# Hagtaril/HiddenPose

Hardware: AMD Instinct MI355X
Metric: samples/sec (128x128x512 meas) fwd+bwd (higher is better)
Workload: dtype f32; 1 GPU; NlosPose train step (fwd+L2Joint+BCEDice loss+bwd+Adam), 128x128x512 transients, batch 4/GPU, fp32, random-init weights, weight gradients of the 3^3 / 4^3 convolutions (and of small 1^3 ones) on a second stream; global_batch=4, world_size=1, parallelism=dp1

## Files before the change

### hiddenpose_amd/_lib.py

```python
from __future__ import annotations

import ctypes as C
import os
import threading

_PKG = os.path.dirname(os.path.abspath(__file__))
LIB_PATH = os.path.join(_PKG, "libhiddenpose_hip.so")

_lock = threading.Lock()
_lib = None


class HiddenPoseHipError(RuntimeError):
    pass


_vp, _fp, _i, _sz, _d = C.c_void_p, C.c_void_p, C.c_int, C.c_size_t, C.c_double
SIGNATURES = {
    "hp_version": (_i, []),
    "hp_last_error_string": (C.c_char_p, []),
    "hp_profile_enable": (_i, [_i]),
    "hp_profile_reset": (_i, []),
    "hp_profile_count": (_i, []),
    "hp_profile_get": (_i, [_i, C.c_char_p, _i, C.POINTER(C.c_int64), C.POINTER(C.c_double)]),
    "hp_range_enable": (_i, [_i]),
    "hp_range_push": (_i, [C.c_char_p]),
    "hp_range_pop": (_i, []),
    "hp_range_start": (C.c_int64, [C.c_char_p]),
    "hp_range_stop": (_i, [C.c_int64]),
    "hp_lct_host_constants": (_i, [_i, _i, _d, _d, _vp, _vp, _vp, _vp, _vp, _vp]),
    "hp_lct_plan_create": (_i, [C.POINTER(_vp), _i, _i, _d, _d, _i, _i]),
    "hp_lct_plan_create_mode": (_i, [C.POINTER(_vp), _i, _i, _d, _d, _i, _i, _i]),
    "hp_lct_plan_destroy": (_i, [_vp]),
    "hp_laplacian5_forward": (_i, [_fp, _fp, _fp, C.c_long, _i, _i, _i, _vp]),
    "hp_laplacian5_backward": (_i, [_fp, _fp, _fp, C.c_long, _i, _i, _i, _vp]),
    "hp_lct_workspace_bytes": (_sz, [_vp, _i]),
    "hp_lct_forward": (_i, [_vp, _fp, _fp, _i, _vp, _sz, _vp]),
    "hp_lct_backward": (_i, [_vp, _fp, _fp, _i, _vp, _sz, _vp]),
    "hp_lct_plan_get_invpsf": (_i, [_vp, _vp, _vp]),
    "hp_conv3d_packed_weight_elems": (_sz, [_vp]),
    "hp_conv3d_pack_weight": (_i, [_vp, _fp, _fp, _fp, _vp]),
    "hp_conv3d_unpack_wgrad": (_i, [_vp, _fp, _fp, _vp]),
    "hp_conv3d_forward": (_i, [_vp, _fp, _fp, _fp, _fp, _vp, _vp]),
    "hp_conv3d_backward_data": (_i, [_vp, _fp, _fp, _fp, _fp, _vp]),
    "hp_conv3d_backward_data_masked": (_i, [_vp, _fp, _fp, _fp, _fp, _vp, _vp]),
    "hp_conv3d_backward_data_bnsums": (_i, [_vp, _fp, _fp, _fp, _fp, _vp, _fp, _fp, _fp, _fp, _fp, _i, _vp, _vp, C.POINTER(C.c_int), _vp]),
    "hp_bn_backward_presummed": (_i, [_fp, _fp, _fp, C.c_long, _i, _fp, _fp, _fp, _fp, _i, _i, _fp, _fp, _vp, _vp, _vp, _i, _vp]),
    "hp_conv3d_backward_weight": (_i, [_vp, _fp, _fp, _fp, _vp]),
    "hp_conv3d_backward_weight_split": (_i, [_vp, C.POINTER(C.c_long), C.POINTER(C.c_long)]),
    "hp_bn_train_finalize": (_i, [_vp, C.c_long, _i, C.c_float, C.c_float, _fp, _fp, _fp, _fp, _vp]),
    "hp_bn_train_finalize_counted": (_i, [_vp, C.c_long, _i, C.c_float, C.c_float, _fp, _fp, _fp, _fp, _vp, _vp]),
    "hp_bn_eval_stats": (_i, [_fp, _fp, _i, C.c_float, _fp, _fp, _vp]),
    "hp_bn_apply": (_i, [_fp, _fp, _fp, C.c_long, _i, _fp, _fp, _fp, _fp, _i, _vp, _i, _vp]),
    "hp_bn_apply_res_bn": (_i, [_fp, _fp, _fp, C.c_long, _i, _fp, _fp, _fp, _fp, _i, _vp, _fp, _fp, _fp, _fp, _i, _vp]),
    "hp_cast_f32_to_bf16": (_i, [_fp, _vp, C.c_long, _vp]),
    "hp_cast_bf16_to_f32": (_i, [_vp, _fp, C.c_long, _vp]),
    "hp_bn_backward_workspace_bytes": (_sz, [_i]),
    "hp_bn_backward_dual": (_i, [_fp, _vp, C.c_long, _i, _fp, _fp, _fp, _fp, _fp, _i, _fp, _fp, _fp, _fp, _fp, _fp, _fp, _i,
                                 _fp, _fp, _vp, _i, _vp]),
    "hp_bn_backward": (_i, [_fp, _fp, _fp, _fp, _fp, C.c_long, _i, _fp, _fp, _fp, _fp, _i, _i, _fp, _fp, _vp, _vp, _i, _vp]),
    "hp_maxpool3d_k3s2_forward": (_i, [_fp, _fp, _i, _i, _i, _i, _i, _vp]),
    "hp_maxpool3d_k3s2_backward": (_i, [_fp, _fp, _fp, _fp, _i, _i, _i, _i, _i, _vp]),
    "hp_layout_transpose": (_i, [_fp, _fp, _i, C.c_long, _i, _i, _vp]),
    "hp_stem_bn_pool_workspace_bytes": (_sz, [_i]),
    "hp_stem_bn_relu_pool_forward": (_i, [_fp, _fp, _i, _i, _i, _i, _i, _fp, _fp, _fp, _fp, _vp, _vp]),
    "hp_stem_bn_relu_pool_backward": (_i, [_fp, _fp, _fp, _fp, _i, _i, _i, _i, _i, _fp, _fp, _fp, _fp, _i, _fp, _fp, _vp, _vp]),
    "hp_dconv3_forward": (_i, [_fp, _fp, _fp, _fp, _i, _i, _i, _i, _i, _i, _i, _vp]),
    "hp_dconv3_forward_fused": (_i, [_fp, _fp, _fp, _fp, _fp, _vp, _i, _i, _i, _i, _i, _i, _i, C.c_float, _vp]),
    "hp_dconv3_backward_data_workspace_bytes": (_sz, [_i, _i, _i, _i, _i, _i]),
    "hp_dconv3_backward_data": (_i, [_fp, _fp, _fp, _i, _i, _i, _i, _i, _i, _i, _vp, _vp]),
    "hp_dconv3_forward_fused_p": (_i, [_fp, _fp, _fp, _fp, _fp, _vp, _i, _i, _i, _i, _i, _i, _i, C.c_float, _i, _vp]),
    "hp_dconv3_backward_data_p": (_i, [_fp, _fp, _fp, _i, _i, _i, _i, _i, _i, _i, _i, _vp, _vp]),
    "hp_dconv3_backward_weight_p": (_i, [_fp, _fp, _fp, _fp, _i, _i, _i, _i, _i, _i, _i, _i, _vp, _vp]),
    "hp_dconv3_backward_weight_workspace_bytes": (_sz, [_i, _i, _i, _i, _i, _i]),
    "hp_dconv3_backward_weight": (_i, [_fp, _fp, _fp, _fp, _i, _i, _i, _i, _i, _i, _i, _vp, _vp]),
    "hp_groupnorm_workspace_bytes": (_sz, [_i, _i]),
    "hp_groupnorm_relu_forward": (_i, [_fp, _fp, _i, _i, _i, C.c_long, _fp, _fp, C.c_float, _fp, _fp, _vp, _vp]),
    "hp_groupnorm_relu_forward_v2": (_i, [_fp, _fp, _i, _i, _i, C.c_long, _fp, _fp, C.c_float, _vp, _fp, _fp, _fp, _fp, _vp, _vp]),
    "hp_groupnorm_relu_backward_v2": (_i, [_fp, _fp, _fp, _i, _i, _i, C.c_long, _fp, _fp, _fp, _fp, _fp, _fp, _fp, _vp, _vp]),
    "hp_maxpool3d_k2_forward": (_i, [_fp, _fp, C.c_long, _i, _i, _i, _vp]),
# ... 148 lines not shown
```

### hiddenpose_amd/csrc/hp_internal.h

```cpp
#pragma once
#include <hip/hip_runtime.h>

#include "hp_host.h"

namespace hp {

#define HP_CHECK_HIP(expr)                                                              \
  do {                                                                                  \
    hipError_t _e = (expr);                                                             \
    if (_e != hipSuccess) {                                                             \
      ::hp::set_error("%s:%d: %s -> %s", __FILE__, __LINE__, #expr, hipGetErrorString(_e)); \
      return HP_ERR_HIP;                                                                \
    }                                                                                   \
  } while (0)

struct ProfScope {
  ProfScope(const char* name, hipStream_t st);
  ~ProfScope();
  int slot = -1;
  hipStream_t st = nullptr;
  hipEvent_t stop = nullptr;
};
#define HP_PROF(name, stream) ::hp::ProfScope _hp_prof_scope(name, stream)

constexpr int ATTN_JOINT_SPLITS = 32;
constexpr int ATTN_GROUPED_MAX_N = 64;
constexpr int ATTN_BWD_DQ_SPLITS = 32;
void launch_attn_bwd_joint_keys(const float* ws_dk, const float* ws_dv, float* dK, float* dV, int BH, int Ntok, int dh, int nj, int frames,
                                hipStream_t st);
void launch_attn_bwd_dq_joint(const float* Q, const float* K0, const float* V, const float* dout, const float* lse, const float* delta,
                              float* part, float* dQ, int BH, int heads, int dh, int Ntok, int nj, hipStream_t st);
void launch_attention_patch(const float* Q, const float* K, const float* V, float* out, float* lse, int B, int heads, int dh, int Ntok,
                            int nj, int n, int frames, hipStream_t st);
void launch_attention_joint_merge(const float* part, float* out, float* lse, int BH, int heads, int dh, int Ntok, int nj, int nsplit,
                                  hipStream_t st);
void launch_attn_bwd_delta(const float* out, const float* dout, float* delta, int B, int heads, int dh, int Ntok, hipStream_t st);
void launch_attn_bwd_dq_patch(const float* Q, const float* K, const float* V, const float* dout, const float* lse, const float* delta,
                              float* dQ, int BH, int heads, int dh, int Ntok, int nj, int n, int frames, hipStream_t st);
void launch_attn_bwd_dq_joint_merge(const float* part, float* dQ, int BH, int Ntok, int dh, int nj, int nsplit, hipStream_t st);
void launch_attention_patch16(const float* Q, const float* K, const float* V, float* out, float* lse, int B, int heads, int dh, int Ntok,
                              int nj, int n, int frames, int precision, hipStream_t st);
void launch_attn_bwd_dq_joint_masked(const float* Q, const float* K0, const float* V, const float* dout, const float* lse,
                                     const float* delta, float* part, float* dQ, int BH, int heads, int dh, int Ntok, int nj,
                                     const unsigned char* key_mask, hipStream_t st);
inline int attn_masked16_check(const char* who, int num_joints, int mask_patch_queries) {
  HP_REQUIRE(mask_patch_queries == 0 || mask_patch_queries == 1, "%s: mask_patch_queries must be 0 or 1", who);
  if (mask_patch_queries) {
    set_error("%s: mask_patch_queries 1 not built at a 16-bit precision (only the joint / class queries apply the mask there)", who);
    return HP_ERR_UNSUPPORTED;
  }
  if (num_joints == 0) {
    set_error("%s: num_joints 0 not built (with no joint / class key an all-masked group would have an empty key set)", who);
    return HP_ERR_UNSUPPORTED;
  }
  return HP_OK;
}

#ifdef __HIPCC__
__device__ __forceinline__ float4 hp_ld4(const void* p, long i, int half) {
  if (half) {
    const uint2 u = *reinterpret_cast<const uint2*>(reinterpret_cast<const unsigned short*>(p) + i);
    return make_float4(__uint_as_float(u.x << 16), __uint_as_float(u.x & 0xffff0000u), __uint_as_float(u.y << 16),
                       __uint_as_float(u.y & 0xffff0000u));
  }
  return *reinterpret_cast<const float4*>(reinterpret_cast<const float*>(p) + i);
}
__device__ __forceinline__ float hp_ld1(const void* p, long i, int half) {
  if (half) return __uint_as_float((unsigned)reinterpret_cast<const unsigned short*>(p)[i] << 16);
  return reinterpret_cast<const float*>(p)[i];
}
__device__ __forceinline__ unsigned short hp_f2bf(float v) {
  typedef __attribute__((ext_vector_type(2))) float hp_f32x2;
  typedef __attribute__((ext_vector_type(2))) __bf16 hp_bf16x2;
  const hp_bf16x2 h = __builtin_convertvector((hp_f32x2){v, 0.f}, hp_bf16x2);
  return __builtin_bit_cast(unsigned int, h) & 0xffffu;
}
__device__ __forceinline__ void hp_st4(void* p, long i, float4 v, int half) {
  if (half) {
    typedef __attribute__((ext_vector_type(2))) float hp_f32x2;
    typedef __attribute__((ext_vector_type(2))) __bf16 hp_bf16x2;
    const hp_bf16x2 lo = __builtin_convertvector((hp_f32x2){v.x, v.y}, hp_bf16x2);
    const hp_bf16x2 hi = __builtin_convertvector((hp_f32x2){v.z, v.w}, hp_bf16x2);
    *reinterpret_cast<uint2*>(reinterpret_cast<unsigned short*>(p) + i) =
        make_uint2(__builtin_bit_cast(unsigned int, lo), __builtin_bit_cast(unsigned int, hi));
    return;
  }
  *reinterpret_cast<float4*>(reinterpret_cast<float*>(p) + i) = v;
}
__device__ __forceinline__ unsigned hp_extent(long total, long base_off, int esz) {
  const long bytes = (total - base_off) * esz;
// ... 10 lines not shown
```

### hiddenpose_amd/csrc/norm_kernels.hip

```cpp
#include <algorithm>
#include <cstdint>
#include <cstdlib>
#include <initializer_list>

#include "hp_internal.h"

namespace hp {

constexpr int ET = 256;
#ifndef HP_BN_UNR_H
#define HP_BN_UNR_H 8
#endif

#ifndef HP_BN_NT
#define HP_BN_NT 1
#endif
typedef float hp_f4v __attribute__((ext_vector_type(4)));
typedef unsigned hp_u4v __attribute__((ext_vector_type(4)));
__device__ __forceinline__ float4 ld_stream(const float4* p) {
#if HP_BN_NT
  const hp_f4v t = __builtin_nontemporal_load(reinterpret_cast<const hp_f4v*>(p));
  return make_float4(t.x, t.y, t.z, t.w);
#else
  return *p;
// ... 1077 lines not shown
  }
  hipLaunchKernelGGL(k_bn_bwd_coef, dim3((C + 127) / 128), dim3(128), 0, st, red, M, C, mean, rstd, gamma, train, dgamma,
                     dbeta, ca, cb, cc);
  {
    HP_PROF("bn_bwd_apply", st);
    const long n4 = M * C4;
    if (bytemask) {
      const int iom = io_mode(C4, {dy_half, z_half, dz_half});
      HP_LAUNCH_IOM(k_bn_bwd_apply_bytemask, iom, grid_for_bwd(n4 / (iom == 1 ? 2 : 1)), st, dy, dy_half, z, z_half, dz, dz_half, n4, C4,
                    (const float4*)ca, (const float4*)cb, (const float4*)cc, relu_mask);
    } else if (remask) {
      const int iom = io_mode(C4, {dy_half, z_half, dz_half});
      HP_LAUNCH_IOM(k_bn_bwd_apply_mask, iom, grid_for_bwd(n4 / (iom == 1 ? 2 : 1)), st, dy, dy_half, z, z_half, dz, dz_half, n4, C4,
                    (const float4*)ca, (const float4*)cb, (const float4*)cc, (const float4*)mean, (const float4*)rstd,
                    (const float4*)gamma, (const float4*)beta_for_mask, relu);
    } else {
      const int iom = io_mode(C4, {z_half, dz_half});
      HP_LAUNCH_IOM(k_bn_bwd_apply, iom, grid_for_bwd(n4 / (iom == 1 ? 2 : 1)), st, (const void*)gbuf, dz_half, z, z_half, dz, dz_half, n4,
                    C4, (const float4*)ca, (const float4*)cb, (const float4*)cc);
    }
  }
  HP_CHECK_HIP(hipGetLastError());
  return HP_OK;
}

__global__ void k_bn_sum_slots(const double* __restrict__ slots, double* __restrict__ red, int n) {
  const int i = blockIdx.x * blockDim.x + threadIdx.x;
  if (i >= n) return;
  double s = 0.0;
  for (int sl = 0; sl < HP_STATS_SLOTS; ++sl) s += slots[(size_t)sl * n + i];
  red[i] = s;
}

extern "C" int hp_bn_backward_presummed(const void* dy, const void* z, void* dz, long M, int C, const float* mean,
                                        const float* rstd, const float* gamma, const float* beta_for_mask, int relu, int train,
                                        float* dgamma, float* dbeta, const unsigned char* relu_mask, const double* sums,
                                        void* workspace, int io, void* stream) {
  const int dy_half = (io & HP_BN_DY_BF16) ? 1 : 0, dz_half = (io & HP_BN_DZ_BF16) ? 1 : 0, z_half = (io & HP_BN_Z_BF16) ? 1 : 0;
  HP_REQUIRE(dy && z && dz && mean && rstd && gamma && sums && workspace && M > 0 && C > 0 && C % 4 == 0 && dy != dz,
             "hp_bn_backward_presummed: bad argument");
  HP_REQUIRE(!relu || relu_mask || beta_for_mask, "hp_bn_backward_presummed: relu needs the byte mask, or beta to rebuild the mask from z");
  hipStream_t st = (hipStream_t)stream;
  double* red = (double*)workspace;
  float* ca = (float*)(red + 2 * C);
  float* cb = ca + C;
  float* cc = cb + C;
  const int C4 = C / 4;
  hipLaunchKernelGGL(k_bn_sum_slots, dim3((2 * C + 127) / 128), dim3(128), 0, st, sums, red, 2 * C);
  hipLaunchKernelGGL(k_bn_bwd_coef, dim3((C + 127) / 128), dim3(128), 0, st, red, M, C, mean, rstd, gamma, train, dgamma,
                     dbeta, ca, cb, cc);
  {
    HP_PROF("bn_bwd_apply", st);
    const long n4 = M * C4;
    const int iom = io_mode(C4, {dy_half, z_half, dz_half});
    if (relu && relu_mask)
      HP_LAUNCH_IOM(k_bn_bwd_apply_bytemask, iom, grid_for_bwd(n4 / (iom == 1 ? 2 : 1)), st, dy, dy_half, z, z_half, dz, dz_half, n4, C4,
                    (const float4*)ca, (const float4*)cb, (const float4*)cc, relu_mask);
    else
      HP_LAUNCH_IOM(k_bn_bwd_apply_mask, iom, grid_for_bwd(n4 / (iom == 1 ? 2 : 1)), st, dy, dy_half, z, z_half, dz, dz_half, n4, C4,
                    (const float4*)ca, (const float4*)cb, (const float4*)cc, (const float4*)mean, (const float4*)rstd,
                    (const float4*)gamma, (const float4*)beta_for_mask, relu);
  }
  HP_CHECK_HIP(hipGetLastError());
  return HP_OK;
}

// ... 169 lines not shown
```

### hiddenpose_amd/hip_ops.py

```python
from __future__ import annotations

import os

import torch
import torch.nn.functional as F

HIP_STAGES = {"feature_extraction", "lct_forward", "lct_backward", "normalize_feature", "unet3d", "posenet3d_50",
              "softmax_integral", "weighted_mse", "bce_dice"}
ATEN_STAGES = {"Adam"}


def _need_cuda(x: torch.Tensor, what: str) -> None:
    if not x.is_cuda:
        from ._lib import HiddenPoseHipError

        raise HiddenPoseHipError(f"{what}: tensor is on {x.device}; this package has no CPU path")


import ctypes as _C

from . import _lib


def _stream(t):
# ... 1057 lines not shown
        x, w, gamma, beta, z, pooled, mean, rstd = ctx.saved_tensors
        desc, train = ctx.cfg
        b, d, h, wd_, cout = z.shape
        dp = dp.contiguous()
        st = _stream(x)
        with torch.cuda.device(x.device):
            if _h(dp):
                dpf = torch.empty_like(dp, dtype=torch.float32)
                _lib.check(L.hp_cast_bf16_to_f32(dp.data_ptr(), dpf.data_ptr(), dp.numel(), st), "hp_cast_bf16_to_f32")
                dp = dpf
            dz = torch.empty_like(z)
            dgamma = torch.empty_like(gamma)
            dbeta = torch.empty_like(gamma)
            ws = torch.empty(int(L.hp_stem_bn_pool_workspace_bytes(cout)) // 4 + 4, dtype=torch.float32, device=x.device)
            _lib.check(L.hp_stem_bn_relu_pool_backward(z.data_ptr(), pooled.data_ptr(), dp.data_ptr(), dz.data_ptr(), b, d, h, wd_,
                                                       cout, mean.data_ptr(), rstd.data_ptr(), gamma.data_ptr(), beta.data_ptr(),
                                                       1 if train else 0, dgamma.data_ptr(), dbeta.data_ptr(), ws.data_ptr(), st),
                       "hp_stem_bn_relu_pool_backward")
            dx, dw = _conv_grads(desc, x, w, dz, ctx.needs_input_grad[0])
        return dx, dw, dgamma, dbeta, None


def stem_conv_bn_relu_pool(x, conv, bn):
    _need_cuda(x, "posenet3d_50")
    b, c, d, h, w = x.shape
    assert c == 1
    return _StemConvBnReluPool.apply(x.reshape(b, d, h, w, 1), conv.weight, bn.weight, bn.bias, bn)


def head_conv_to_ncdhw(x, conv, bn_in=None):
    return _ConvBiasToNCDHW.apply(x, conv.weight, conv.bias, bn_in)


class _SoftArgmax(torch.autograd.Function):
    @staticmethod
    def forward(ctx, preds, num_joints, W, H, D):
        _need_cuda(preds, "softmax_integral")
        heat = preds.contiguous()
        B = heat.shape[0]
        bj = B * num_joints
        assert heat.numel() == bj * D * H * W
        joints = torch.empty(B, num_joints * 3, dtype=torch.float32, device=heat.device)
        stat = torch.empty(bj * 2, dtype=torch.float32, device=heat.device)
        with torch.cuda.device(heat.device):
            _lib.check(_lib.lib().hp_softargmax_forward(heat.data_ptr(), joints.data_ptr(), stat.data_ptr(), bj, D, H, W,
                                                        _stream(heat)), "hp_softargmax_forward")
        ctx.save_for_backward(heat, joints, stat)
        ctx.dims = (bj, D, H, W)
        return joints

    @staticmethod
    def backward(ctx, gj):
        heat, joints, stat = ctx.saved_tensors
        bj, D, H, W = ctx.dims
        dheat = torch.empty_like(heat)
        with torch.cuda.device(heat.device):
            _lib.check(_lib.lib().hp_softargmax_backward(heat.data_ptr(), joints.data_ptr(), stat.data_ptr(),
                                                         gj.contiguous().data_ptr(), dheat.data_ptr(), bj, D, H, W,
                                                         _stream(heat)), "hp_softargmax_backward")
        return dheat, None, None, None, None


def softmax_integral(preds, num_joints, W, H, D):
    return _SoftArgmax.apply(preds, num_joints, W, H, D)


# ... 142 lines not shown
```

### hiddenpose_amd/posenet3d_50.py

```python
from __future__ import annotations

import torch
from torch import nn

from . import _lib
from . import hip_ops as ops

LAYERS = (3, 4, 6, 3)
PLANES = (64, 128, 256, 512)


class Bottleneck(nn.Module):
    expansion = 4

    def __init__(self, in_planes, planes, stride=1, downsample=None):
        super().__init__()
        self.conv1 = nn.Conv3d(in_planes, planes, 1, bias=False)
        self.bn1 = nn.BatchNorm3d(planes)
        self.conv2 = nn.Conv3d(planes, planes, 3, stride=stride, padding=1, bias=False)
        self.bn2 = nn.BatchNorm3d(planes)
        self.conv3 = nn.Conv3d(planes, planes * 4, 1, bias=False)
        self.bn3 = nn.BatchNorm3d(planes * 4)
        self.downsample = downsample
        self.stride = stride
# ... 13 lines not shown
        if self.downsample is not None:
            if link is not None:
                link.arrivals = 2
            return ops.conv_bn_act(o, self.conv3, self.bn3, relu=True, residual=res, res_link=rl, bn_in=b2)
        if link is not None:
            link.arrivals = 1
        b3 = ops.bn_link() if (link is not None and ops._BN_FUSE_RES) else None
        y = ops.conv_bn_act(o, self.conv3, self.bn3, relu=True, residual=x, link_out=link, bn_in=b2, bn_out=b3)
        ops.offer_res_bn(y, b3)
        return y


class DeconvHead(nn.Module):
    def __init__(self, in_channels, num_layers, num_filters, kernel_size, conv_kernel_size, num_joints):
        super().__init__()
        assert kernel_size == 4 and conv_kernel_size == 1
        self.features = nn.ModuleList()
        for i in range(num_layers):
            cin = in_channels if i == 0 else num_filters
            self.features.append(nn.ConvTranspose3d(cin, num_filters, 4, stride=2, padding=1, bias=False))
            self.features.append(nn.BatchNorm3d(num_filters))
            self.features.append(nn.Identity())
        self.features.append(nn.Conv3d(num_filters, num_joints, 1, bias=True))
        for m in self.modules():
            if isinstance(m, (nn.Conv3d, nn.ConvTranspose3d)):
                nn.init.normal_(m.weight, mean=0, std=0.001)
                if getattr(m, "bias", None) is not None:
                    nn.init.constant_(m.bias, 0)

    def forward(self, x):
        f = self.features
        prev = ops.take_res_bn(x)
        for i in range(0, len(f) - 1, 3):
            nxt = ops.bn_link()
            x = ops.deconv_bn_relu(x, f[i], f[i + 1], bn_in=prev, bn_out=nxt)
            prev = nxt
        return ops.head_conv_to_ncdhw(x, f[-1], prev)


class ResNet(nn.Module):
    conv_precision = "fp32"

    def __init__(self, n_input_channels=1):
        super().__init__()
        _lib.lib()
        self.in_planes = 64
        self.conv1 = nn.Conv3d(n_input_channels, 64, 7, stride=1, padding=3, bias=False)
        self.bn1 = nn.BatchNorm3d(64)
        self.layer1 = self._make_layer(PLANES[0], LAYERS[0], 1)
        self.layer2 = self._make_layer(PLANES[1], LAYERS[1], 2)
        self.layer3 = self._make_layer(PLANES[2], LAYERS[2], 2)
        self.layer4 = self._make_layer(PLANES[3], LAYERS[3], 2)
        self.head = DeconvHead(2048, 3, 256, 4, 1, 24)
        for m in self.modules():
            if isinstance(m, nn.Conv3d):
                nn.init.kaiming_normal_(m.weight, mode="fan_out", nonlinearity="relu")
            elif isinstance(m, nn.BatchNorm3d):
                nn.init.constant_(m.weight, 1)
                nn.init.constant_(m.bias, 0)

    def _make_layer(self, planes, blocks, stride):
        ds = None
        if stride != 1 or self.in_planes != planes * 4:
            ds = nn.Sequential(nn.Conv3d(self.in_planes, planes * 4, 1, stride=stride, bias=False),
                               nn.BatchNorm3d(planes * 4))
        layers = [Bottleneck(self.in_planes, planes, stride, ds)]
# ... 20 lines not shown
```

### include/hiddenpose_hip.h

```cpp
#ifndef HIDDENPOSE_HIP_H
#define HIDDENPOSE_HIP_H

#include <stddef.h>
#include <stdint.h>

#ifdef __cplusplus
extern "C" {
#endif

typedef enum hp_status {
  HP_OK = 0,
  HP_ERR_BAD_ARG = -1,
  HP_ERR_UNSUPPORTED = -2,
  HP_ERR_HIP = -3,
  HP_ERR_WORKSPACE = -4,
  HP_ERR_NO_DEVICE = -5
} hp_status;

int hp_version(void);
const char* hp_last_error_string(void);

int hp_profile_enable(int on);
int hp_profile_reset(void);
int hp_profile_count(void);
// ... 60 lines not shown
                            const void* addend, void* stream);
int hp_conv3d_backward_data_masked(const hp_conv_desc* d, const void* dy, const float* w_dgrad, void* dx,
                                   const void* addend, const unsigned char* addend_mask, void* stream);
int hp_conv3d_backward_data_bnsums(const hp_conv_desc* d, const void* dy, const float* w_dgrad, void* dx, const void* addend,
                                   const unsigned char* addend_mask, const float* z, const float* mean, const float* rstd,
                                   const float* gamma, const float* beta, int relu, const unsigned char* relu_mask, double* sums,
                                   int* fused, void* stream);
int hp_conv3d_backward_weight(const hp_conv_desc* d, const void* x, const void* dy, float* dw_packed, void* stream);
int hp_conv3d_backward_weight_split(const hp_conv_desc* d, long* msplit, long* chunk_rows);

#define HP_BN_ACT_BF16 1
#define HP_BN_DY_BF16 2
#define HP_BN_DZ_BF16 4
#define HP_BN_Z_BF16 8
int hp_bn_train_finalize(const double* stats, long M, int C, float eps, float momentum, float* mean, float* rstd,
                         float* running_mean, float* running_var, void* stream);
int hp_bn_train_finalize_counted(const double* stats, long M, int C, float eps, float momentum, float* mean, float* rstd,
                                 float* running_mean, float* running_var, long long* num_batches_tracked, void* stream);
int hp_bn_eval_stats(const float* running_mean, const float* running_var, int C, float eps, float* mean, float* rstd,
                     void* stream);
int hp_bn_apply(const void* z, const void* res, void* y, long M, int C, const float* mean, const float* rstd,
                const float* gamma, const float* beta, int relu, unsigned char* relu_mask, int io, void* stream);
int hp_bn_apply_res_bn(const void* z, const void* res, void* y, long M, int C, const float* mean, const float* rstd,
                       const float* gamma, const float* beta, int relu, unsigned char* relu_mask, const float* res_mean,
                       const float* res_rstd, const float* res_gamma, const float* res_beta, int io, void* stream);
size_t hp_bn_backward_workspace_bytes(int C);
int hp_bn_backward(const void* dy, const float* y, const void* z, void* g_out, void* dz, long M, int C,
                   const float* mean, const float* rstd, const float* gamma, const float* beta_for_mask, int relu,
                   int train, float* dgamma, float* dbeta, const unsigned char* relu_mask, void* workspace, int io,
                   void* stream);
int hp_bn_backward_presummed(const void* dy, const void* z, void* dz, long M, int C, const float* mean, const float* rstd,
                             const float* gamma, const float* beta_for_mask, int relu, int train, float* dgamma, float* dbeta,
                             const unsigned char* relu_mask, const double* sums, void* workspace, int io, void* stream);
int hp_bn_backward_dual(const void* dy, const unsigned char* relu_mask, long M, int C, const void* z_a, void* dz_a,
                        const float* mean_a, const float* rstd_a, const float* gamma_a, int train_a, float* dgamma_a,
                        float* dbeta_a, const void* z_b, void* dz_b, const float* mean_b, const float* rstd_b,
                        const float* gamma_b, int train_b, float* dgamma_b, float* dbeta_b, void* workspace, int io,
                        void* stream);
int hp_cast_f32_to_bf16(const float* x, void* y, long n, void* stream);
int hp_cast_bf16_to_f32(const void* x, float* y, long n, void* stream);
int hp_maxpool3d_k3s2_forward(const float* x, float* y, int B, int D, int H, int W, int C, void* stream);
int hp_maxpool3d_k3s2_backward(const float* x, const float* y, const float* dy, float* dx, int B, int D, int H, int W,
                               int C, void* stream);
size_t hp_stem_bn_pool_workspace_bytes(int C);
int hp_stem_bn_relu_pool_forward(const float* z, float* pooled, int B, int D, int H, int W, int C, const float* mean,
                                 const float* rstd, const float* gamma, const float* beta, void* workspace, void* stream);
int hp_stem_bn_relu_pool_backward(const float* z, const float* pooled, const float* dpooled, float* dz, int B, int D, int H,
                                  int W, int C, const float* mean, const float* rstd, const float* gamma, const float* beta,
                                  int train, float* dgamma, float* dbeta, void* workspace, void* stream);
int hp_layout_transpose(const float* in, float* out, int B, long V, int C, int to_channels_first, void* stream);

int hp_dconv3_forward(const float* x, const float* w, const float* bias, float* y, int B, int cin, int cout, int D,
                      int H, int W, int replicate_pad, void* stream);
int hp_dconv3_forward_fused(const float* x, const float* w, const float* bias, const float* residual, float* y,
                            double* stats, int B, int cin, int cout, int D, int H, int W, int replicate_pad, float slope,
                            void* stream);
size_t hp_dconv3_backward_data_workspace_bytes(int B, int cin, int D, int H, int W, int replicate_pad);
int hp_dconv3_backward_data(const float* gy, const float* w, float* gx, int B, int cin, int cout, int D, int H, int W,
                            int replicate_pad, void* workspace, void* stream);
int hp_dconv3_forward_fused_p(const float* x, const float* w, const float* bias, const float* residual, float* y,
                              double* stats, int B, int cin, int cout, int D, int H, int W, int replicate_pad, float slope,
                              int precision, void* stream);
int hp_dconv3_backward_data_p(const float* gy, const float* w, float* gx, int B, int cin, int cout, int D, int H, int W,
                              int replicate_pad, int precision, void* workspace, void* stream);
int hp_dconv3_backward_weight_p(const float* x, const float* gy, float* dw, float* dbias, int B, int cin, int cout, int D,
                                int H, int W, int replicate_pad, int precision, void* workspace, void* stream);
// ... 173 lines not shown
```

Before: 8.712 samples/s.

## Fuse last deconv BN+ReLU with 1x1x1 heatmap head conv in forward and backward

Adds HIP kernels that apply the final deconv's BatchNorm+ReLU on the fly and immediately run the 1x1x1 joint-heatmap convolution with MFMA. The backward path recomputes the activation from z, fusing the head weight/bias gradients, BN reduction sums and the dz application. This avoids materialising the BN output, separate 1x1 conv kernels and layout transposes for the large final feature map. In exchange it adds multi-pass reduction kernels with per-workgroup partials and recomputation of the activation.

```diff
diff --git a/hiddenpose_amd/_lib.py b/hiddenpose_amd/_lib.py
--- a/hiddenpose_amd/_lib.py
+++ b/hiddenpose_amd/_lib.py
@@ -46,6 +46,10 @@
     "hp_conv3d_backward_data_masked": (_i, [_vp, _fp, _fp, _fp, _fp, _vp, _vp]),
     "hp_conv3d_backward_data_bnsums": (_i, [_vp, _fp, _fp, _fp, _fp, _vp, _fp, _fp, _fp, _fp, _fp, _i, _vp, _vp, C.POINTER(C.c_int), _vp]),
     "hp_bn_backward_presummed": (_i, [_fp, _fp, _fp, C.c_long, _i, _fp, _fp, _fp, _fp, _i, _i, _fp, _fp, _vp, _vp, _vp, _i, _vp]),
+    "hp_head_bn_forward": (_i, [_fp, _fp, _fp, _fp, C.c_long, C.c_long, _i, _i, _fp, _fp, _fp, _fp, C.POINTER(C.c_int), _vp]),
+    "hp_head_bn_backward_workspace_bytes": (_sz, [_i, _i]),
+    "hp_head_bn_backward": (_i, [_fp, _fp, _fp, _fp, _fp, _fp, C.c_long, C.c_long, _i, _i, _fp, _fp, _fp, _fp, _i, _fp, _fp, _vp,
+                                 C.POINTER(C.c_int), _vp]),
     "hp_conv3d_backward_weight": (_i, [_vp, _fp, _fp, _fp, _vp]),
     "hp_conv3d_backward_weight_split": (_i, [_vp, C.POINTER(C.c_long), C.POINTER(C.c_long)]),
     "hp_bn_train_finalize": (_i, [_vp, C.c_long, _i, C.c_float, C.c_float, _fp, _fp, _fp, _fp, _vp]),
diff --git a/hiddenpose_amd/csrc/head_kernels.hip b/hiddenpose_amd/csrc/head_kernels.hip
--- /dev/null
+++ b/hiddenpose_amd/csrc/head_kernels.hip
@@ -0,0 +1,496 @@
+#include <algorithm>
+#include <cstdlib>
+#include <mutex>
+
+#include "hiddenpose_hip.h"
+#include "hp_internal.h"
+
+namespace hp {
+
+typedef float hd_f32x16 __attribute__((ext_vector_type(16)));
+typedef float hd_f4v __attribute__((ext_vector_type(4)));
+
+constexpr int HT = 256;
+constexpr int HM = 128;
+constexpr int HK = 64;
+constexpr int ZLD = HK + 4;
+constexpr int DLD = 33;
+constexpr int HEAD_CW = 128;
+constexpr int HEAD_MAX_WGS = 512;
+
+__device__ __forceinline__ float4 hd_ld_nt(const float* p) {
+  const hd_f4v t = __builtin_nontemporal_load(reinterpret_cast<const hd_f4v*>(p));
+  return make_float4(t.x, t.y, t.z, t.w);
+}
+__device__ __forceinline__ void hd_st_nt(float* p, float4 v) {
+  __builtin_nontemporal_store((hd_f4v){v.x, v.y, v.z, v.w}, reinterpret_cast<hd_f4v*>(p));
+}
+__device__ __forceinline__ int hd_acc_row(int r, int half) { return 8 * (r >> 2) + 4 * half + (r & 3); }
+
+__global__ __launch_bounds__(HT) void k_head_bn_fwd(const float* __restrict__ z, const float* __restrict__ w,
+                                                    const float* __restrict__ bias, float* __restrict__ heat, long M, long V, int C,
+                                                    int J, const float* __restrict__ mean, const float* __restrict__ rstd,
+                                                    const float* __restrict__ gamma, const float* __restrict__ beta) {
+  extern __shared__ float4 hd_smem[];
+  float* sm = reinterpret_cast<float*>(hd_smem);
+  const int WLD = C + 4;
+  float* Wp = sm;
+  float* Y = Wp + 32 * WLD;
+  float* sc = Y + HM * ZLD;
+  float* sh = sc + C;
+  float* sb = sh + C;
+  const int tid = threadIdx.x, lane = tid & 63, wave = tid >> 6, half = lane >> 5, l32 = lane & 31;
+  for (int i = tid; i < 32 * C; i += HT) {
+    const int j = i / C, c = i - j * C, o = c & 7;
+    Wp[j * WLD + (c & ~7) + ((o & 1) ? 4 + (o >> 1) : (o >> 1))] = j < J ? w[(long)j * C + c] : 0.f;
+  }
+  for (int c = tid; c < C; c += HT) {
+    const float s = rstd[c] * gamma[c];
+    sc[c] = s;
+    sh[c] = beta[c] - mean[c] * s;
+  }
+  if (tid < 32) sb[tid] = tid < J ? bias[tid] : 0.f;
+  __syncthreads();
+  const int q = tid & 15, r0 = tid >> 4;
+  const long tiles = (M + HM - 1) / HM;
+  const int nch = C / HK;
+  float4 zr[8];
+  auto fetch = [&](long tile, int ch) {
+#pragma unroll
+    for (int i = 0; i < 8; ++i) {
+      const long row = tile * HM + r0 + 16 * i;
+      zr[i] = row < M ? hd_ld_nt(z + row * C + ch * HK + 4 * q) : make_float4(0.f, 0.f, 0.f, 0.f);
+    }
+  };
+  long tile = blockIdx.x;
+  int ch = 0;
+  if (tile < tiles) fetch(tile, 0);
+  hd_f32x16 acc;
+#pragma unroll
+  for (int r = 0; r < 16; ++r) acc[r] = 0.f;
+  const int ycol = 8 * (q >> 1) + 2 * (q & 1);
+  while (tile < tiles) {
+    const float4 s4 = *reinterpret_cast<const float4*>(sc + ch * HK + 4 * q);
+    const float4 t4 = *reinterpret_cast<const float4*>(sh + ch * HK + 4 * q);
+#pragma unroll
+    for (int i = 0; i < 8; ++i) {
+      const float4 v = zr[i];
+      const float y0 = fmaxf(fmaf(v.x, s4.x, t4.x), 0.f), y1 = fmaxf(fmaf(v.y, s4.y, t4.y), 0.f);
+      const float y2 = fmaxf(fmaf(v.z, s4.z, t4.z), 0.f), y3 = fmaxf(fmaf(v.w, s4.w, t4.w), 0.f);
+      float* dst = Y + (r0 + 16 * i) * ZLD + ycol;
+      *reinterpret_cast<float2*>(dst) = make_float2(y0, y2);
+      *reinterpret_cast<float2*>(dst + 4) = make_float2(y1, y3);
+    }
+    long nt = tile;
+    int nc = ch + 1;
+    if (nc == nch) {
+      nc = 0;
+      nt += gridDim.x;
+    }
+    if (nt < tiles) fetch(nt, nc);
+    __syncthreads();
+    const float* ap = Wp + l32 * WLD + ch * HK + 4 * half;
+    const float* bp = Y + (32 * wave + l32) * ZLD + 4 * half;
+#pragma unroll
+    for (int g = 0; g < 8; ++g) {
+      const float4 a4 = *reinterpret_cast<const float4*>(ap + 8 * g);
+      const float4 b4 = *reinterpret_cast<const float4*>(bp + 8 * g);
+      acc = __builtin_amdgcn_mfma_f32_32x32x2f32(a4.x, b4.x, acc, 0, 0, 0);
+      acc = __builtin_amdgcn_mfma_f32_32x32x2f32(a4.y, b4.y, acc, 0, 0, 0);
+      acc = __builtin_amdgcn_mfma_f32_32x32x2f32(a4.z, b4.z, acc, 0, 0, 0);
+      acc = __builtin_amdgcn_mfma_f32_32x32x2f32(a4.w, b4.w, acc, 0, 0, 0);
+    }
+    __syncthreads();
+    if (ch == nch - 1) {
+      const long row = tile * HM + 32 * wave + l32;
+      if (row < M) {
+        const long b = row / V, v = row - b * V;
+        float* hp = heat + b * J * V + v;
+#pragma unroll
+        for (int r = 0; r < 16; ++r) {
+          const int j = hd_acc_row(r, half);
+          if (j < J) hp[(long)j * V] = acc[r] + sb[j];
+        }
+      }
+#pragma unroll
+      for (int r = 0; r < 16; ++r) acc[r] = 0.f;
+    }
+    tile = nt;
+    ch = nc;
+  }
+}
+
+
+template <int NCH>
+__global__ __launch_bounds__(HT) void k_head_bn_bwd_reduce(const float* __restrict__ z, const float* __restrict__ dheat,
+                                                           const float* __restrict__ w, long M, long V, int C, int J, int c0,
+                                                           const float* __restrict__ mean, const float* __restrict__ rstd,
+                                                           const float* __restrict__ gamma, const float* __restrict__ beta,
+                                                           double* __restrict__ sums, float* __restrict__ dw_part,
+                                                           float* __restrict__ db_part) {
+  extern __shared__ float4 hd_smem[];
+  float* sm = reinterpret_cast<float*>(hd_smem);
+  constexpr int CW = NCH * HK;
+  float* Wn = sm;
+  float* Z = Wn + 32 * CW;
+  float* DH = Z + HM * ZLD;
+  float* sc = DH + HM * DLD;
+  float* sh = sc + CW;
+  float* mu = sh + CW;
+  float* rs = mu + CW;
+  const int tid = threadIdx.x, lane = tid & 63, wave = tid >> 6, half = lane >> 5, l32 = lane & 31;
+  for (int i = tid; i < 32 * CW; i += HT) {
+    const int j = i / CW, c = i - j * CW;
+    Wn[i] = j < J ? w[(long)j * C + c0 + c] : 0.f;
+  }
+  for (int c = tid; c < CW; c += HT) {
+    const float m = mean[c0 + c], r = rstd[c0 + c];
+    const float s = r * gamma[c0 + c];
+    sc[c] = s;
+    sh[c] = beta[c0 + c] - m * s;
+    mu[c] = m;
+    rs[c] = r;
+  }
+  const int q = tid & 15, r0 = tid >> 4;
+  const long tiles = (M + HM - 1) / HM;
+  float4 zr[8];
+  auto fetch = [&](long tile, int ch) {
+#pragma unroll
+    for (int i = 0; i < 8; ++i) {
+      const long row = tile * HM + r0 + 16 * i;
+      zr[i] = row < M ? hd_ld_nt(z + row * C + c0 + ch * HK + 4 * q) : make_float4(0.f, 0.f, 0.f, 0.f);
+    }
+  };
+  const int drow = tid & 127, dj0 = tid >> 7;
+  float dhr[16];
+  auto fetch_dh = [&](long tile) {
+    const long row = tile * HM + drow;
+    const bool ok = row < M;
+    const long b = ok ? row / V : 0, v = ok ? row - b * V : 0;
+    const float* p = dheat + b * J * V + v;
+#pragma unroll
+    for (int i = 0; i < 16; ++i) {
+      const int j = dj0 + 2 * i;
+      dhr[i] = (ok && j < J) ? p[(long)j * V] : 0.f;
+    }
+  };
+  long tile = blockIdx.x;
+  if (tile < tiles) {
+    fetch_dh(tile);
+    fetch(tile, 0);
+  }
+  hd_f32x16 aw[NCH][2];
+  float S[NCH][2], Dt[NCH][2];
+#pragma unroll
+  for (int ch = 0; ch < NCH; ++ch)
+#pragma unroll
+    for (int blk = 0; blk < 2; ++blk) {
+      S[ch][blk] = Dt[ch][blk] = 0.f;
+#pragma unroll
+      for (int t = 0; t < 16; ++t) aw[ch][blk][t] = 0.f;
+    }
+  float dbacc = 0.f;
+  const int dbj = tid & 31, dbr = (tid >> 5) * 16;
+  __syncthreads();
+  while (tile < tiles) {
+#pragma unroll
+    for (int i = 0; i < 16; ++i) DH[drow * DLD + dj0 + 2 * i] = dhr[i];
+    __syncthreads();
+    float dhA[16], dhT[16];
+#pragma unroll
+    for (int k = 0; k < 16; ++k) {
+      dhA[k] = DH[(32 * wave + l32) * DLD + 2 * k + half];
+      dhT[k] = DH[(32 * wave + hd_acc_row(k, half)) * DLD + l32];
+    }
+    if (db_part) {
+#pragma unroll
+      for (int i = 0; i < 16; ++i) dbacc += DH[(dbr + i) * DLD + dbj];
+    }
+    const long ntile = tile + gridDim.x;
+    if (ntile < tiles) fetch_dh(ntile);
+#pragma unroll
+    for (int ch = 0; ch < NCH; ++ch) {
+#pragma unroll
+      for (int i = 0; i < 8; ++i) *reinterpret_cast<float4*>(Z + (r0 + 16 * i) * ZLD + 4 * q) = zr[i];
+      if (ch + 1 < NCH) fetch(tile, ch + 1);
+      else if (ntile < tiles) fetch(ntile, 0);
+      __syncthreads();
+#pragma unroll
+      for (int blk = 0; blk < 2; ++blk) {
+        const int cl = ch * HK + blk * 32 + l32;
+        hd_f32x16 acc;
+#pragma unroll
+        for (int r = 0; r < 16; ++r) acc[r] = 0.f;
+#pragma unroll
+        for (int k = 0; k < 16; ++k) acc = __builtin_amdgcn_mfma_f32_32x32x2f32(dhA[k], Wn[(2 * k + half) * CW + cl], acc, 0, 0, 0);
+        const float scv = sc[cl], shv = sh[cl], m = mu[cl], r = rs[cl];
+        float ps = 0.f, pd = 0.f, y[16];
+#pragma unroll
+        for (int t = 0; t < 16; ++t) {
+          const float zv = Z[(32 * wave + hd_acc_row(t, half)) * ZLD + blk * 32 + l32];
+          const float yy = fmaxf(fmaf(zv, scv, shv), 0.f);
+          const float g = yy > 0.f ? acc[t] : 0.f;
+          ps += g;
+          pd += g * (zv - m) * r;
+          y[t] = yy;
+        }
+        S[ch][blk] += ps;
+        Dt[ch][blk] += pd;
+#pragma unroll
+        for (int t = 0; t < 16; ++t) aw[ch][blk] = __builtin_amdgcn_mfma_f32_32x32x2f32(dhT[t], y[t], aw[ch][blk], 0, 0, 0);
+      }
+      __syncthreads();
+    }
+    tile = ntile;
+  }
+  float* DWA = Z;
+  float* SDs = DH;
+#pragma unroll
+  for (int wv = 0; wv < 4; ++wv) {
+    if (wave == wv) {
+#pragma unroll
+      for (int ch = 0; ch < NCH; ++ch)
+#pragma unroll
+        for (int blk = 0; blk < 2; ++blk) {
+          const int cl = ch * HK + blk * 32 + l32;
+#pragma unroll
+          for (int t = 0; t < 16; ++t) {
+            const int idx = hd_acc_row(t, half) * CW + cl;
+            DWA[idx] = (wv ? DWA[idx] : 0.f) + aw[ch][blk][t];
+          }
+          const float s = S[ch][blk] + __shfl_xor(S[ch][blk], 32), d = Dt[ch][blk] + __shfl_xor(Dt[ch][blk], 32);
+          const int si = half * CW + cl;
+          SDs[si] = (wv ? SDs[si] : 0.f) + (half ? d : s);
+        }
+    }
+    __syncthreads();
+  }
+  double* slot = sums + (size_t)(blockIdx.x % HP_STATS_SLOTS) * 2 * C;
+  for (int c = tid; c < CW; c += HT) {
+    atomicAdd(slot + c0 + c, (double)SDs[c]);
+    atomicAdd(slot + C + c0 + c, (double)SDs[CW + c]);
+  }
+  for (int i = tid; i < J * CW; i += HT) {
+    const int j = i / CW, c = i - j * CW;
+    dw_part[((size_t)blockIdx.x * J + j) * C + c0 + c] = DWA[i];
+  }
+  if (db_part) {
+    __syncthreads();
+    SDs[tid] = dbacc;
+    __syncthreads();
+    if (tid < 32) {
+      float s = 0.f;
+#pragma unroll
+      for (int i = 0; i < 8; ++i) s += SDs[tid + 32 * i];
+      db_part[(size_t)blockIdx.x * 32 + tid] = s;
+    }
+  }
+}
+
+__global__ void k_head_dw_finalize(const float* __restrict__ dw_part, const float* __restrict__ db_part, int parts, int C, int J,
+                                   float* __restrict__ dw, float* __restrict__ db) {
+  const int i = blockIdx.x * blockDim.x + threadIdx.x;
+  const int n = J * C;
+  if (i < n) {
+    double s = 0.0;
+    for (int p = 0; p < parts; ++p) s += (double)dw_part[(size_t)p * n + i];
+    dw[i] = (float)s;
+  } else if (i < n + J) {
+    const int j = i - n;
+    double s = 0.0;
+    for (int p = 0; p < parts; ++p) s += (double)db_part[(size_t)p * 32 + j];
+    db[j] = (float)s;
+  }
+}
+
+__global__ __launch_bounds__(HT) void k_head_bn_bwd_apply(const float* __restrict__ z, const float* __restrict__ dheat,
+                                                          const float* __restrict__ w, float* __restrict__ dz, long M, long V, int C,
+                                                          int J, const float* __restrict__ mean, const float* __restrict__ rstd,
+                                                          const float* __restrict__ gamma, const float* __restrict__ beta,
+                                                          const float* __restrict__ ca, const float* __restrict__ cb,
+                                                          const float* __restrict__ cc) {
+  extern __shared__ float4 hd_smem[];
+  float* sm = reinterpret_cast<float*>(hd_smem);
+  float* Wn = sm;
+  float* Z = Wn + 32 * C;
+  float* sc = Z + HM * ZLD;
+  float* sh = sc + C;
+  float* ka = sh + C;
+  float* kb = ka + C;
+  float* kc = kb + C;
+  const int tid = threadIdx.x, lane = tid & 63, wave = tid >> 6, half = lane >> 5, l32 = lane & 31;
+  for (int i = tid; i < 32 * C; i += HT) Wn[i] = i < J * C ? w[i] : 0.f;
+  for (int c = tid; c < C; c += HT) {
+    const float s = rstd[c] * gamma[c];
+    sc[c] = s;
+    sh[c] = beta[c] - mean[c] * s;
+    ka[c] = ca[c];
+    kb[c] = cb[c];
+    kc[c] = cc[c];
+  }
+  const int q = tid & 15, r0 = tid >> 4;
+  const long tiles = (M + HM - 1) / HM;
+  const int nch = C / HK;
+  float4 zr[8];
+  auto fetch = [&](long tile, int ch) {
+#pragma unroll
+    for (int i = 0; i < 8; ++i) {
+      const long row = tile * HM + r0 + 16 * i;
+      zr[i] = row < M ? hd_ld_nt(z + row * C + ch * HK + 4 * q) : make_float4(0.f, 0.f, 0.f, 0.f);
+    }
+  };
+  float dhn[16];
+  auto fetch_dh = [&](long tile) {
+    const long row = tile * HM + 32 * wave + l32;
+    const bool ok = row < M;
+    const long b = ok ? row / V : 0, v = ok ? row - b * V : 0;
+    const float* p = dheat + b * J * V + v;
+#pragma unroll
+    for (int k = 0; k < 16; ++k) {
+      const int j = 2 * k + half;
+      dhn[k] = (ok && j < J) ? p[(long)j * V] : 0.f;
+    }
+  };
+  long tile = blockIdx.x;
+  if (tile < tiles) {
+    fetch_dh(tile);
+    fetch(tile, 0);
+  }
+  __syncthreads();
+  while (tile < tiles) {
+    float dhA[16];
+#pragma unroll
+    for (int k = 0; k < 16; ++k) dhA[k] = dhn[k];
+    const long ntile = tile + gridDim.x;
+    if (ntile < tiles) fetch_dh(ntile);
+    for (int ch = 0; ch < nch; ++ch) {
+#pragma unroll
+      for (int i = 0; i < 8; ++i) *reinterpret_cast<float4*>(Z + (r0 + 16 * i) * ZLD + 4 * q) = zr[i];
+      if (ch + 1 < nch) fetch(tile, ch + 1);
+      else if (ntile < tiles) fetch(ntile, 0);
+      __syncthreads();
+#pragma unroll
+      for (int blk = 0; blk < 2; ++blk) {
+        const int cl = ch * HK + blk * 32 + l32;
+        hd_f32x16 acc;
+#pragma unroll
+        for (int r = 0; r < 16; ++r) acc[r] = 0.f;
+#pragma unroll
+        for (int k = 0; k < 16; ++k) acc = __builtin_amdgcn_mfma_f32_32x32x2f32(dhA[k], Wn[(2 * k + half) * C + cl], acc, 0, 0, 0);
+        const float scv = sc[cl], shv = sh[cl], a = ka[cl], b = kb[cl], k0 = kc[cl];
+#pragma unroll
+        for (int t = 0; t < 16; ++t) {
+          float* zp = Z + (32 * wave + hd_acc_row(t, half)) * ZLD + blk * 32 + l32;
+          const float zv = *zp;
+          const float g = fmaf(zv, scv, shv) > 0.f ? acc[t] : 0.f;
+          *zp = a * g + b * zv + k0;
+        }
+      }
+      __syncthreads();
+#pragma unroll
+      for (int i = 0; i < 8; ++i) {
+        const long row = tile * HM + r0 + 16 * i;
+        if (row < M) hd_st_nt(dz + row * C + ch * HK + 4 * q, *reinterpret_cast<const float4*>(Z + (r0 + 16 * i) * ZLD + 4 * q));
+      }
+      __syncthreads();
+    }
+    tile = ntile;
+  }
+}
+
+static unsigned head_grid(long tiles, long dflt) {
+  static const long env = getenv("HP_HEAD_GRID") ? atol(getenv("HP_HEAD_GRID")) : 0;
+  const long cap = std::min<long>(env > 0 ? env : dflt, HEAD_MAX_WGS);
+  return (unsigned)std::max<long>(1, std::min<long>(tiles, cap));
+}
+
+static bool head_geometry_ok(int C, int J) { return C > 0 && C % 64 == 0 && C <= 512 && J >= 1 && J <= 32; }
+
+static size_t head_fwd_lds(int C) { return sizeof(float) * ((size_t)32 * (C + 4) + HM * ZLD + 2 * C + 32); }
+static size_t head_red_lds(int CW) { return sizeof(float) * ((size_t)32 * CW + HM * ZLD + HM * DLD + 4 * CW); }
+static size_t head_app_lds(int C) { return sizeof(float) * ((size_t)32 * C + HM * ZLD + 5 * C); }
+
+static hipError_t head_lds_opt_in() {
+  static std::once_flag once;
+  static hipError_t rc = hipSuccess;
+  std::call_once(once, [&] {
+    rc = hipFuncSetAttribute((const void*)k_head_bn_fwd, hipFuncAttributeMaxDynamicSharedMemorySize, (int)head_fwd_lds(512));
+    if (rc == hipSuccess)
+      rc = hipFuncSetAttribute((const void*)k_head_bn_bwd_reduce<2>, hipFuncAttributeMaxDynamicSharedMemorySize, (int)head_red_lds(128));
+    if (rc == hipSuccess)
+      rc = hipFuncSetAttribute((const void*)k_head_bn_bwd_apply, hipFuncAttributeMaxDynamicSharedMemorySize, (int)head_app_lds(512));
+  });
+  return rc;
+}
+
+}
+
+using namespace hp;
+
+extern "C" int hp_head_bn_forward(const float* z, const float* w, const float* bias, float* heat, long rows, long voxels, int C,
+                                  int J, const float* mean, const float* rstd, const float* gamma, const float* beta, int* fused,
+                                  void* stream) {
+  HP_REQUIRE(fused, "hp_head_bn_forward: fused must not be NULL");
+  *fused = 0;
+  HP_REQUIRE(z && w && bias && heat && mean && rstd && gamma && beta, "hp_head_bn_forward: null pointer");
+  HP_REQUIRE(rows > 0 && voxels > 0 && rows % voxels == 0 && C > 0 && J > 0, "hp_head_bn_forward: bad size");
+  if (!head_geometry_ok(C, J)) return HP_OK;
+  hipStream_t st = (hipStream_t)stream;
+  HP_CHECK_HIP(head_lds_opt_in());
+  const long tiles = (rows + HM - 1) / HM;
+  HP_PROF("head_bn_fwd", st);
+  hipLaunchKernelGGL(k_head_bn_fwd, dim3(head_grid(tiles, 512)), dim3(HT), head_fwd_lds(C), st, z, w, bias, heat, rows, voxels, C, J,
+                     mean, rstd, gamma, beta);
+  HP_CHECK_HIP(hipGetLastError());
+  *fused = 1;
+  return HP_OK;
+}
+
+extern "C" size_t hp_head_bn_backward_workspace_bytes(int C, int J) {
+  if (!head_geometry_ok(C, J)) return 0;
+  return sizeof(double) * ((size_t)HP_STATS_SLOTS * 2 * C + 2 * C) + sizeof(float) * ((size_t)3 * C + (size_t)HEAD_MAX_WGS * ((size_t)J * C + 32));
+}
+
+extern "C" int hp_head_bn_backward(const float* z, const float* dheat, const float* w, float* dz, float* dw, float* dbias, long rows,
+                                   long voxels, int C, int J, const float* mean, const float* rstd, const float* gamma,
+                                   const float* beta, int train, float* dgamma, float* dbeta, void* workspace, int* fused,
+                                   void* stream) {
+  HP_REQUIRE(fused, "hp_head_bn_backward: fused must not be NULL");
+  *fused = 0;
+  HP_REQUIRE(z && dheat && w && dz && dw && dbias && mean && rstd && gamma && beta && workspace, "hp_head_bn_backward: null pointer");
+  HP_REQUIRE(rows > 0 && voxels > 0 && rows % voxels == 0 && C > 0 && J > 0, "hp_head_bn_backward: bad size");
+  HP_REQUIRE(z != dz, "hp_head_bn_backward: dz must not alias z");
+  if (!head_geometry_ok(C, J)) return HP_OK;
+  hipStream_t st = (hipStream_t)stream;
+  HP_CHECK_HIP(head_lds_opt_in());
+  double* slots = (double*)workspace;
+  double* red = slots + (size_t)HP_STATS_SLOTS * 2 * C;
+  float* ca = (float*)(red + 2 * C);
+  float* cb = ca + C;
+  float* cc = cb + C;
+  float* dw_part = cc + C;
+  const long tiles = (rows + HM - 1) / HM;
+  const unsigned gr = head_grid(tiles, 256);
+  float* db_part = dw_part + (size_t)gr * J * C;
+  HP_CHECK_HIP(hipMemsetAsync(slots, 0, sizeof(double) * HP_STATS_SLOTS * 2 * C, st));
+  {
+    HP_PROF("head_bn_bwd_reduce", st);
+    for (int c0 = 0; c0 < C; c0 += HEAD_CW) {
+      const int nch = std::min(HEAD_CW, C - c0) / HK;
+      auto kern = nch == 1 ? k_head_bn_bwd_reduce<1> : k_head_bn_bwd_reduce<2>;
+      hipLaunchKernelGGL(kern, dim3(gr), dim3(HT), head_red_lds(nch * HK), st, z, dheat, w, rows, voxels, C, J, c0, mean, rstd, gamma,
+                         beta, slots, dw_part, c0 == 0 ? db_part : (float*)nullptr);
+    }
+  }
+  hipLaunchKernelGGL(k_head_dw_finalize, dim3((unsigned)((J * C + J + 255) / 256)), dim3(256), 0, st, (const float*)dw_part,
+                     (const float*)db_part, (int)gr, C, J, dw, dbias);
+  launch_bn_slots_coef(slots, red, rows, C, mean, rstd, gamma, train, dgamma, dbeta, ca, cb, cc, st);
+  {
+    HP_PROF("head_bn_bwd_apply", st);
+    hipLaunchKernelGGL(k_head_bn_bwd_apply, dim3(head_grid(tiles, 512)), dim3(HT), head_app_lds(C), st, z, dheat, w, dz, rows, voxels, C,
+                       J, mean, rstd, gamma, beta, (const float*)ca, (const float*)cb, (const float*)cc);
+  }
+  HP_CHECK_HIP(hipGetLastError());
+  *fused = 1;
+  return HP_OK;
+}
diff --git a/hiddenpose_amd/csrc/hp_internal.h b/hiddenpose_amd/csrc/hp_internal.h
--- a/hiddenpose_amd/csrc/hp_internal.h
+++ b/hiddenpose_amd/csrc/hp_internal.h
@@ -56,6 +56,9 @@
   return HP_OK;
 }
 
+void launch_bn_slots_coef(const double* slots, double* red, long M, int C, const float* mean, const float* rstd, const float* gamma,
+                          int train, float* dgamma, float* dbeta, float* ca, float* cb, float* cc, hipStream_t st);
+
 #ifdef __HIPCC__
 __device__ __forceinline__ float4 hp_ld4(const void* p, long i, int half) {
   if (half) {
diff --git a/hiddenpose_amd/csrc/norm_kernels.hip b/hiddenpose_amd/csrc/norm_kernels.hip
--- a/hiddenpose_amd/csrc/norm_kernels.hip
+++ b/hiddenpose_amd/csrc/norm_kernels.hip
@@ -1133,6 +1133,13 @@
   red[i] = s;
 }
 
+void hp::launch_bn_slots_coef(const double* slots, double* red, long M, int C, const float* mean, const float* rstd, const float* gamma,
+                              int train, float* dgamma, float* dbeta, float* ca, float* cb, float* cc, hipStream_t st) {
+  hipLaunchKernelGGL(k_bn_sum_slots, dim3((2 * C + 127) / 128), dim3(128), 0, st, slots, red, 2 * C);
+  hipLaunchKernelGGL(k_bn_bwd_coef, dim3((C + 127) / 128), dim3(128), 0, st, (const double*)red, M, C, mean, rstd, gamma, train, dgamma,
+                     dbeta, ca, cb, cc);
+}
+
 extern "C" int hp_bn_backward_presummed(const void* dy, const void* z, void* dz, long M, int C, const float* mean,
                                         const float* rstd, const float* gamma, const float* beta_for_mask, int relu, int train,
                                         float* dgamma, float* dbeta, const unsigned char* relu_mask, const double* sums,
diff --git a/hiddenpose_amd/hip_ops.py b/hiddenpose_amd/hip_ops.py
--- a/hiddenpose_amd/hip_ops.py
+++ b/hiddenpose_amd/hip_ops.py
@@ -1113,6 +1113,103 @@
     return _ConvBiasToNCDHW.apply(x, conv.weight, conv.bias, bn_in)
 
 
+_HEAD_FUSE = __import__("os").environ.get("HP_HEAD_FUSE", "1") != "0"
+_head_fused_calls = [0]
+
+
+def head_fusable(x, deconv, bn, conv) -> bool:
+    if not _HEAD_FUSE or _conv_precision != 0 or _act_bf16 or x.dtype != torch.float32 or conv.bias is None:
+        return False
+    if conv.kernel_size != (1, 1, 1) or conv.stride != (1, 1, 1) or conv.padding != (0, 0, 0) or not bn.affine:
+        return False
+    if int(_lib.lib().hp_head_bn_backward_workspace_bytes(conv.in_channels, conv.out_channels)) == 0:
+        return False
+    if not torch.is_grad_enabled():
+        return True
+    need = [x.requires_grad or deconv.weight.requires_grad or bn.weight.requires_grad or bn.bias.requires_grad,
+            conv.weight.requires_grad, conv.bias.requires_grad]
+    return all(need) or not any(need)
+
+
+class _DeconvBnReluHead(torch.autograd.Function):
+
+    @staticmethod
+    def forward(ctx, x, w, gamma, beta, hw, hb, bn, bn_in=None):
+        L = _lib.lib()
+        x = x.contiguous()
+        ctx.use_epoch = _use_epoch[0]
+        cout, J = w.shape[1], hw.shape[0]
+        desc = _desc(x, cout, 4, 2, 1, True)
+        do, ho, wo = _out_dims(desc)
+        st = _stream(x)
+        with torch.cuda.device(x.device):
+            wf, _ = _pack(desc, w, True, False, False)
+            z = torch.empty(desc.B, do, ho, wo, cout, dtype=torch.float32, device=x.device)
+            M = z.numel() // cout
+            train = bn.training
+            stats = torch.empty(_lib.STATS_SLOTS * 2 * cout, dtype=torch.float64, device=x.device) if train else None
+            desc.io = 0
+            _lib.check(L.hp_conv3d_forward(_C.byref(desc), x.data_ptr(), wf.data_ptr(), None, z.data_ptr(),
+                                           _lib.ptr(stats), st), "hp_conv3d_forward")
+            mean = torch.empty(cout, dtype=torch.float32, device=x.device)
+            rstd = torch.empty_like(mean)
+            if train:
+                mom = 0.1 if bn.momentum is None else bn.momentum
+                _lib.check(L.hp_bn_train_finalize_counted(stats.data_ptr(), M, cout, bn.eps, mom, mean.data_ptr(), rstd.data_ptr(),
+                                                          bn.running_mean.data_ptr(), bn.running_var.data_ptr(),
+                                                          bn.num_batches_tracked.data_ptr(), st), "hp_bn_train_finalize")
+            else:
+                _lib.check(L.hp_bn_eval_stats(bn.running_mean.data_ptr(), bn.running_var.data_ptr(), cout, bn.eps,
+                                              mean.data_ptr(), rstd.data_ptr(), st), "hp_bn_eval_stats")
+            hw_c, gamma_c, beta_c = hw.detach().contiguous(), gamma.detach().contiguous(), beta.detach().contiguous()
+            heat = torch.empty(desc.B, J, do, ho, wo, dtype=torch.float32, device=x.device)
+            fused = _C.c_int(0)
+            _lib.check(L.hp_head_bn_forward(z.data_ptr(), hw_c.data_ptr(), hb.detach().contiguous().data_ptr(), heat.data_ptr(), M,
+                                            do * ho * wo, cout, J, mean.data_ptr(), rstd.data_ptr(), gamma_c.data_ptr(),
+                                            beta_c.data_ptr(), _C.byref(fused), st), "hp_head_bn_forward")
+            if not fused.value:
+                raise _lib.HiddenPoseHipError(f"hp_head_bn_forward: C = {cout}, J = {J} not fused")
+        _head_fused_calls[0] += 1
+        ctx.save_for_backward(x, w, gamma, beta, z, mean, rstd, hw)
+        ctx.cfg = (desc, train)
+        ctx.bn_in = bn_in
+        return heat
+
+    @staticmethod
+    def backward(ctx, dheat):
+        L = _lib.lib()
+        x, w, gamma, beta, z, mean, rstd, hw = ctx.saved_tensors
+        desc, train = ctx.cfg
+        cout, J = z.shape[-1], hw.shape[0]
+        M = z.numel() // cout
+        dheat = dheat.contiguous()
+        st = _stream(x)
+        with torch.cuda.device(x.device):
+            dz = torch.empty_like(z)
+            dhw = torch.empty_like(hw, memory_format=torch.contiguous_format)
+            dhb = torch.empty(J, dtype=torch.float32, device=x.device)
+            dgamma = torch.empty_like(gamma)
+            dbeta = torch.empty_like(gamma)
+            ws = torch.empty(int(L.hp_head_bn_backward_workspace_bytes(cout, J)) // 8 + 1, dtype=torch.float64, device=x.device)
+            fused = _C.c_int(0)
+            _lib.check(L.hp_head_bn_backward(z.data_ptr(), dheat.data_ptr(), hw.contiguous().data_ptr(), dz.data_ptr(), dhw.data_ptr(),
+                                             dhb.data_ptr(), M, M // desc.B, cout, J, mean.data_ptr(), rstd.data_ptr(),
+                                             gamma.contiguous().data_ptr(), beta.contiguous().data_ptr(), 1 if train else 0,
+                                             dgamma.data_ptr(), dbeta.data_ptr(), ws.data_ptr(), _C.byref(fused), st),
+                       "hp_head_bn_backward")
+            if not fused.value:
+                raise _lib.HiddenPoseHipError(f"hp_head_bn_backward: C = {cout}, J = {J} not fused")
+            dx, dw = _conv_grads(desc, x, w, dz, ctx.needs_input_grad[0], bn_in=ctx.bn_in,
+                                 force_main=_WGRAD_ASYNC and _shared_use(ctx, w))
+        return dx, dw, dgamma, dbeta, dhw, dhb, None, None
+
+
+def deconv_bn_relu_head(x, deconv, bn, conv, bn_in=None):
+    if _WGRAD_ASYNC:
+        _note_use(deconv.weight)
+    return _DeconvBnReluHead.apply(x, deconv.weight, bn.weight, bn.bias, conv.weight, conv.bias, bn, bn_in)
+
+
 class _SoftArgmax(torch.autograd.Function):
     @staticmethod
     def forward(ctx, preds, num_joints, W, H, D):
diff --git a/hiddenpose_amd/posenet3d_50.py b/hiddenpose_amd/posenet3d_50.py
--- a/hiddenpose_amd/posenet3d_50.py
+++ b/hiddenpose_amd/posenet3d_50.py
@@ -69,6 +69,8 @@
         f = self.features
         prev = ops.take_res_bn(x)
         for i in range(0, len(f) - 1, 3):
+            if i == len(f) - 4 and ops.head_fusable(x, f[i], f[i + 1], f[-1]):
+                return ops.deconv_bn_relu_head(x, f[i], f[i + 1], f[-1], bn_in=prev)
             nxt = ops.bn_link()
             x = ops.deconv_bn_relu(x, f[i], f[i + 1], bn_in=prev, bn_out=nxt)
             prev = nxt
diff --git a/include/hiddenpose_hip.h b/include/hiddenpose_hip.h
--- a/include/hiddenpose_hip.h
+++ b/include/hiddenpose_hip.h
@@ -116,6 +116,12 @@
 int hp_bn_backward_presummed(const void* dy, const void* z, void* dz, long M, int C, const float* mean, const float* rstd,
                              const float* gamma, const float* beta_for_mask, int relu, int train, float* dgamma, float* dbeta,
                              const unsigned char* relu_mask, const double* sums, void* workspace, int io, void* stream);
+int hp_head_bn_forward(const float* z, const float* w, const float* bias, float* heat, long rows, long voxels, int C, int J,
+                       const float* mean, const float* rstd, const float* gamma, const float* beta, int* fused, void* stream);
+size_t hp_head_bn_backward_workspace_bytes(int C, int J);
+int hp_head_bn_backward(const float* z, const float* dheat, const float* w, float* dz, float* dw, float* dbias, long rows,
+                        long voxels, int C, int J, const float* mean, const float* rstd, const float* gamma, const float* beta,
+                        int train, float* dgamma, float* dbeta, void* workspace, int* fused, void* stream);
 int hp_bn_backward_dual(const void* dy, const unsigned char* relu_mask, long M, int C, const void* z_a, void* dz_a,
                         const float* mean_a, const float* rstd_a, const float* gamma_a, int train_a, float* dgamma_a,
                         float* dbeta_a, const void* z_b, void* dz_b, const float* mean_b, const float* rstd_b,
```

Result: no change. 8.792 samples/s (median of 6 runs) (+0.9%).
